# manoskary/analysisgnn

Hardware: AMD Instinct MI355X
Metric: subgraph-nodes/sec fwd+bwd, HybridGNN L=3 H=256 (higher is better)
Workload: dtype f32; 1 GPU; C2 (sampled, the batch a training step sees): HybridGNN L=3 H=256 out=128, 21 task heads, 32 neighbour-sampled subgraphs x (500 target notes + [5,5] hops) per GPU, per-hop counts passed (every layer trimmed); 16335 notes, 104099 edges per GPU; train step = fwd + objective (wloss) + bwd + allreduce + clip + AdamW, CSR rebuilt every step; hipGraph replay; workload_id=c2s, per_gpu_subgraphs=32, objective=wloss, parallelism=dp1, allreduce=none (one rank)

## Files before the change

analysisgnn_amd/_lib.py:

```python
from __future__ import annotations

import ctypes as C
import os
from typing import Optional, Sequence

import torch

from . import resident

_HERE = os.path.dirname(os.path.abspath(__file__))
LIB_PATH = os.path.join(_HERE, "libagnn_hip.so")
MAX_SEG = 32

SPMM_MEAN, SPMM_SKIP_SELF, SPMM_ACCUM = 1, 2, 4
INT32_MAX = 2 ** 31 - 1


class AgnnError(RuntimeError):
    pass


class CooSeg(C.Structure):
    _fields_ = [("row", C.c_void_p), ("col", C.c_void_p), ("etype", C.c_void_p),
                ("etype_code", C.c_int64), ("n_edges", C.c_int64), ("n_rows", C.c_int64)]
# ... 163 lines not shown
    "agnn_sample_members": (C.c_int, [C.c_void_p, C.c_int64, C.c_void_p, C.c_void_p, C.c_void_p, C.c_int32, C.c_int32, C.c_int32,
                                      C.POINTER(C.c_int32), C.c_int32, C.c_void_p, C.c_void_p, C.c_void_p, C.c_void_p]),
    "agnn_sample_compact_nodes": (C.c_int64, [C.POINTER(Sampler), C.POINTER(C.c_int32)]),
    "agnn_sample_compact": (C.c_int, [C.POINTER(Sampler), C.POINTER(C.c_int32), C.c_void_p, C.c_void_p, C.c_void_p]),
    "agnn_gather_rows_f32": (C.c_int, [C.c_void_p, C.c_int64, C.c_void_p, C.c_int64, C.c_int32, C.c_void_p, C.c_int64, C.c_void_p]),
    "agnn_gather_i64": (C.c_int, [C.c_void_p, C.c_int64, C.c_void_p, C.c_int64, C.c_int32, C.c_int64, C.c_void_p, C.c_int64, C.c_void_p]),
    "agnn_relt_fwd_f32": (C.c_int, [C.c_int, C.POINTER(ReltItem), C.c_int32, C.c_int32, C.c_int32, C.c_int64, C.c_void_p]),
    "agnn_relt_bwd_f32": (C.c_int, [C.c_int, C.POINTER(ReltItem), C.c_int32, C.c_int32, C.c_int32, C.c_int64, C.c_void_p]),
    "agnn_relt_dw_workspace_bytes": (C.c_size_t, [C.c_int, C.c_int32, C.c_int32, C.c_int32, C.c_int64]),
    "agnn_relt_dw_f32": (C.c_int, [C.c_int, C.POINTER(ReltItem), C.c_int32, C.c_int32, C.c_int32, C.c_int64, C.c_void_p, C.c_size_t,
                                  C.c_void_p]),
    "agnn_wgrad_batch_workspace_bytes": (C.c_size_t, [C.c_int32, C.POINTER(WgradItem)]),
    "agnn_wgrad_batch_f32": (C.c_int, [C.c_int32, C.POINTER(WgradItem), C.c_void_p, C.c_size_t, C.c_void_p]),
    "agnn_grad_epilogue_workspace_bytes": (C.c_size_t, [C.c_int32, C.POINTER(GradItem)]),
    "agnn_grad_epilogue_f32": (C.c_int, [C.c_int32, C.POINTER(GradItem), C.c_int32, C.POINTER(ColsumItem), C.c_void_p, C.c_size_t, C.c_void_p]),
    "agnn_gemm_nt_f32": (C.c_int, [C.c_void_p, C.c_int64, C.c_void_p, C.c_int64, C.c_void_p, C.c_int64, C.c_int32, C.c_int32, C.c_void_p,
                                   C.c_int64, C.c_void_p]),
    "agnn_gemm_nn_f32": (C.c_int, [C.c_void_p, C.c_int64, C.c_void_p, C.c_int64, C.c_void_p, C.c_int64, C.c_int32, C.c_int32, C.c_void_p,
                                   C.c_int64, C.c_void_p]),
    "agnn_gemm_nt2_f32": (C.c_int, [C.c_void_p, C.c_int64, C.c_int32, C.c_void_p, C.c_int64, C.c_int32, C.c_void_p, C.c_int64, C.c_void_p,
                                    C.c_int64, C.c_int32, C.c_void_p, C.c_int64, C.c_void_p]),
    "agnn_pool_cat_norm_f32": (C.c_int, [C.POINTER(Rel), C.c_void_p, C.c_int64, C.c_int64, C.c_int64, C.c_int32, C.c_int32, C.c_void_p,
                                         C.c_void_p, C.c_float, C.c_void_p, C.c_int64, C.c_void_p, C.c_int64, C.c_void_p, C.c_void_p,
                                         C.c_void_p, C.c_void_p]),
    "agnn_pool_cat_bwd_f32": (C.c_int, [C.POINTER(Rel), C.c_void_p, C.c_int64, C.c_void_p, C.c_int64, C.c_int64, C.c_int32, C.c_void_p,
                                        C.c_int64, C.c_void_p]),
    "agnn_absdiff_fwd_f32": (C.c_int, [C.c_void_p, C.c_void_p, C.c_void_p, C.c_int64, C.c_int64, C.c_int32, C.c_void_p, C.c_void_p, C.c_int64,
                                       C.c_void_p]),
    "agnn_absdiff_bwd_f32": (C.c_int, [C.c_void_p, C.c_void_p, C.c_void_p, C.c_int64, C.c_int64, C.c_int32, C.c_void_p, C.c_void_p, C.c_int64,
                                       C.c_int32, C.c_int32, C.c_void_p, C.c_int64, C.c_void_p]),
# ... 199 lines not shown
```

analysisgnn_amd/csrc/wgrad.hip:

```cpp
#include "agnn_common.h"

namespace {

typedef float f32x16 __attribute__((ext_vector_type(16)));

struct WgArgs {
  const float* dy;
  const float* x;
  int64_t ld_dy, ld_x;
  int32_t n, out_f, in_f;
  int32_t rows_per_slice;
  int32_t tiles_in;
  float* slab;
  float* slab_b;
  int32_t out_pad, in_pad;
};

__device__ __forceinline__ void wgrad_tile(const WgArgs& a, const int tile, const int slice) {
  const int lane = threadIdx.x & 63;
  const int wave = threadIdx.x >> 6;
  const int wm = wave >> 1, wn = wave & 1;
  const int to = tile / a.tiles_in, ti = tile - to * a.tiles_in;
  const int kk = lane >> 5, c32 = lane & 31;
  const int ocol = to * 128 + wm * 64 + 2 * c32;
// ... 480 lines not shown
  int32_t item, c0, c1;
};

bool spans_overlap(const EpiSpan& a, const EpiSpan& b) {
  const float* a_end = a.p + static_cast<int64_t>(a.rows - 1) * a.ld + a.cols;
  const float* b_end = b.p + static_cast<int64_t>(b.rows - 1) * b.ld + b.cols;
  if (a_end <= b.p || b_end <= a.p) return false;
  if (a.rows > 1 && b.rows > 1 && a.ld == b.ld) {
    int64_t r = (b.p - a.p) % a.ld;
    if (r < 0) r += a.ld;
    if (r >= a.cols && r + b.cols <= a.ld) return false;
  }
  return true;
}

}

static void epi_as_wgrad(int32_t n_items, const agnn_grad_item_t* items, agnn_wgrad_item_t* out) {
  for (int i = 0; i < n_items; ++i) {
    const agnn_grad_item_t& g = items[i];
    out[i] = agnn_wgrad_item_t{g.dy, g.x, nullptr, nullptr, g.ld_dy, g.ld_x, g.in_f, g.n, g.out_f, g.in_f};
  }
}

extern "C" size_t agnn_grad_epilogue_workspace_bytes(int32_t n_items, const agnn_grad_item_t* items) {
  if (n_items <= 0 || n_items > kWgBatchMax || !items) return 0;
  agnn_wgrad_item_t w[kWgBatchMax];
  epi_as_wgrad(n_items, items, w);
  return agnn_wgrad_batch_workspace_bytes(n_items, w);
}
// ... 5 lines not shown
  if (n_sums < 0 || n_sums > kEpiSumMax || (n_sums > 0 && !sums)) return fail(AGNN_EINVAL, "grad_epilogue: %d column sums (0 .. %d)", n_sums, kEpiSumMax);
  if (n_items == 0 && n_sums == 0) return AGNN_OK;
  BatchPlan bp;
  bp.n = 0;
  bp.total_floats = 0;
  float* ws = nullptr;
  if (n_items > 0) {
    agnn_wgrad_item_t w[kWgBatchMax];
    epi_as_wgrad(n_items, items, w);
    if (int rc = batch_plan(n_items, w, bp)) return rc;
    if (!workspace || workspace_bytes < bp.total_floats * sizeof(float) + 256) return fail(AGNN_ENOMEM, "grad_epilogue: workspace too small");
    ws = reinterpret_cast<float*>((reinterpret_cast<uintptr_t>(workspace) + 255) & ~uintptr_t{255});
  }
  static thread_local EpiSpan spans[kWgBatchMax * 2 * AGNN_PACK_MAX_SRC + 2 * kEpiSumMax];
  int n_spans = 0;
  for (int i = 0; i < n_items; ++i) {
    const agnn_grad_item_t& it = items[i];
    if ((it.out_f & 1) || (it.in_f & 1) || (it.ld_dy & 1) || (it.ld_x & 1)) return fail(AGNN_EALIGN, "grad_epilogue: item %d: widths and leading dimensions must be even", i);
    if (!it.dy || !it.x) return fail(AGNN_EINVAL, "grad_epilogue: item %d: null argument", i);
    if ((reinterpret_cast<uintptr_t>(it.dy) | reinterpret_cast<uintptr_t>(it.x)) & 7u) return fail(AGNN_EALIGN, "grad_epilogue: item %d: pointers must be 8-byte aligned", i);
    if (it.ld_dy < it.out_f || it.ld_x < it.in_f) return fail(AGNN_EINVAL, "grad_epilogue: item %d: leading dimension smaller than the width", i);
    if ((static_cast<int64_t>(bp.rps[i]) + 128) * (it.ld_dy > it.ld_x ? it.ld_dy : it.ld_x) * 4 >= (int64_t{1} << 32))
      return fail(AGNN_EINVAL, "grad_epilogue: item %d: a row slice (%d rows x ld) exceeds the kernel's 32-bit byte offsets", i, bp.rps[i]);
    if (it.n_dw < 0 || it.n_dw > AGNN_PACK_MAX_SRC || it.n_db < 0 || it.n_db > AGNN_PACK_MAX_SRC || it.n_dw + it.n_db == 0)
      return fail(AGNN_EINVAL, "grad_epilogue: item %d: %d weight and %d bias destinations (0 .. %d each, one at least)", i, it.n_dw, it.n_db, AGNN_PACK_MAX_SRC);
    for (int k = 0; k < it.n_dw; ++k) {
      const agnn_grad_dst_t& d = it.dw[k];
      const int cols = d.c1 - d.c0;
      if (!d.p || d.c0 < 0 || cols <= 0 || d.c1 > it.in_f || d.ld < cols || d.ld >= (int64_t{1} << 31))
        return fail(AGNN_EINVAL, "grad_epilogue: item %d: destination %d: columns [%d, %d) of %d, ld %lld", i, k, d.c0, d.c1, it.in_f, (long long)d.ld);
      if (reinterpret_cast<uintptr_t>(d.p) & 3u) return fail(AGNN_EALIGN, "grad_epilogue: item %d: destination %d is not a float pointer", i, k);
      if (!(cols & 1) && ((d.c0 & 1) || (d.ld & 1) || (reinterpret_cast<uintptr_t>(d.p) & 7u)))
        return fail(AGNN_EALIGN, "grad_epilogue: item %d: destination %d: an even column block needs an even c0, an even ld and an 8-byte aligned pointer", i, k);
      spans[n_spans++] = EpiSpan{d.p, d.ld, it.out_f, cols, i, d.c0, d.c1};
    }
    for (int k = 0; k < it.n_db; ++k) {
      if (!it.db[k]) return fail(AGNN_EINVAL, "grad_epilogue: item %d: null bias destination %d", i, k);
      if (reinterpret_cast<uintptr_t>(it.db[k]) & 3u) return fail(AGNN_EALIGN, "grad_epilogue: item %d: bias destination %d is not a float pointer", i, k);
      spans[n_spans++] = EpiSpan{it.db[k], it.out_f, 1, it.out_f, -1, 0, 0};
    }
  }
  for (int i = 0; i < n_sums; ++i) {
    const agnn_colsum_item_t& it = sums[i];
    if (it.n <= 0 || it.H <= 0 || (it.H & 3) || it.H > 2048 || !it.workspace || !it.dgamma || !it.dbeta)
      return fail(AGNN_EINVAL, "grad_epilogue: column sum %d: bad sizes or null argument", i);
    if (it.workspace_bytes < static_cast<size_t>(kEpiPartRows) * 2 * it.H * sizeof(float)) return fail(AGNN_ENOMEM, "grad_epilogue: column sum %d: workspace too small", i);
    if ((reinterpret_cast<uintptr_t>(it.dgamma) | reinterpret_cast<uintptr_t>(it.dbeta) | reinterpret_cast<uintptr_t>(it.workspace)) & 3u)
      return fail(AGNN_EALIGN, "grad_epilogue: column sum %d: misaligned", i);
    spans[n_spans++] = EpiSpan{it.dgamma, it.H, 1, it.H, -1, 0, 0};
    spans[n_spans++] = EpiSpan{it.dbeta, it.H, 1, it.H, -1, 0, 0};
  }
  for (int a = 0; a < n_spans; ++a)
    for (int c = a + 1; c < n_spans; ++c) {
      const EpiSpan &sa = spans[a], &sc = spans[c];
      if (sa.item >= 0 && sa.item == sc.item && sa.c0 == sc.c0 && sa.c1 == sc.c1 && sa.p == sc.p && sa.ld == sc.ld) continue;
      if (spans_overlap(sa, sc)) return fail(AGNN_EINVAL, "grad_epilogue: destinations %d and %d of the call overlap", a, c);
    }
  hipStream_t s = static_cast<hipStream_t>(stream_);
  if (n_items > 0) {
    WgBatch wb{};
    wb.n = n_items;
    int wg = 0;
    for (int i = 0; i < n_items; ++i) {
      const agnn_grad_item_t& it = items[i];
      const int out_pad = bp.tiles_out[i] * 128, in_pad = bp.tiles_in[i] * 128;
      wb.it[i] = WgArgs{it.dy, it.x, it.ld_dy, it.ld_x, static_cast<int32_t>(it.n), it.out_f, it.in_f, bp.rps[i], bp.tiles_in[i], ws + bp.slab_off[i],
                        it.n_db > 0 ? ws + bp.slabb_off[i] : nullptr, out_pad, in_pad};
      wb.tiles[i] = bp.tiles_out[i] * bp.tiles_in[i];
      wb.first[i] = wg;
      wg += wb.tiles[i] * bp.S[i];
    }
    wb.first[n_items] = wg;
// ... 2 lines not shown
  }
  int at = 0;
  do {
    EpiBatch eb{};
    int n = 0, n_rec = 0, n_db = 0, blocks = 0;
    while (at < n_items && n_rec + items[at].n_dw <= kEpiRecMax && n_db + items[at].n_db <= kEpiDbMax) {
      const agnn_grad_item_t& it = items[at];
      EpiItem& e = eb.it[n];
      e.slab = ws + bp.slab_off[at];
      e.slab_b = it.n_db > 0 ? ws + bp.slabb_off[at] : nullptr;
      e.S = bp.S[at];
      e.out_f = it.out_f;
      e.in_f = it.in_f;
      e.out_pad = bp.tiles_out[at] * 128;
      e.in_pad = bp.tiles_in[at] * 128;
      e.rec0 = static_cast<int16_t>(n_rec);
      for (int k = 0; k < it.n_dw; ++k) {
        const agnn_grad_dst_t& d = it.dw[k];
        eb.rec[n_rec++] = EpiRec{d.p, static_cast<int32_t>(d.ld), d.c0, d.c1, (d.c1 - d.c0) & 1};
      }
      e.rec1 = static_cast<int16_t>(n_rec);
      e.db0 = static_cast<int16_t>(n_db);
      for (int k = 0; k < it.n_db; ++k) eb.db[n_db++] = it.db[k];
      e.db1 = static_cast<int16_t>(n_db);
      eb.first[n] = blocks;
      int64_t rb = (static_cast<int64_t>(it.out_f) * (it.in_f >> 1) + 31) / 32;
      if (rb > 1024) rb = 1024;
      blocks += static_cast<int>(rb);
      ++n;
      ++at;
    }
    eb.n_items = n;
    if (at == n_items)
      for (int i = 0; i < n_sums; ++i) {
        const agnn_colsum_item_t& it = sums[i];
        int nb = static_cast<int>((it.n + 3) / 4);
        if (nb > kEpiPartRows) nb = kEpiPartRows;
        eb.sum[i] = EpiSum{static_cast<const float*>(it.workspace), it.dgamma, it.dbeta, nb, it.H};
        eb.first[n++] = blocks;
// ... 12 lines not shown
```

analysisgnn_amd/heads.py:

```python
from __future__ import annotations

from typing import Dict, List, Optional, Sequence, Tuple

import torch
import torch.nn as nn
import torch.nn.functional as F

from . import _lib, resident
from .fused import grouped_norm_act
from .linear import all_steal, defer, deferring, grad_slot_groups, leaf_refs, linear, mark_wgrad_async, slot_group, wgrad_stream
from .params import cat_rows, stack_rows


def fused_head_logits(clf_dict: nn.ModuleDict, x: torch.Tensor, tasks: Sequence[str]) -> Tuple[torch.Tensor, List[int]]:
    mods = [clf_dict[t] for t in tasks]
    T = len(mods)
    h2 = mods[0][0].out_features
    W1 = _cat_params([m[0].weight for m in mods])
    b1 = _cat_params([m[0].bias for m in mods])
    gamma = _cat_params([m[2].weight for m in mods], stack=True)
    beta = _cat_params([m[2].bias for m in mods], stack=True)
    offs = [0]
    for m in mods:
        offs.append(offs[-1] + m[3].out_features)
    b2 = _cat_params([m[3].bias for m in mods])
# ... 278 lines not shown
def multitask_cross_entropy(logits: torch.Tensor, offs: Sequence[int], labels: torch.Tensor, label_smoothing: float = 0.1,
                            ignore_index: int = -1) -> torch.Tensor:
    full = len(offs) > 1 and offs[0] == 0 and offs[-1] == logits.shape[1] and all(offs[i] < offs[i + 1] for i in range(len(offs) - 1))
    return _MultiTaskCE.apply(logits, labels, _offs_tensor(offs, logits.device), label_smoothing, ignore_index, full)


def _check_labels(labels: torch.Tensor, T: int, N: int) -> torch.Tensor:
    if labels.dtype != torch.int64:
        raise _lib.AgnnError(f"labels must be int64 (torch.long), got {labels.dtype}")
    if tuple(labels.shape) != (T, N):
        raise _lib.AgnnError(f"labels must have shape [T={T}, N={N}] (one row per task), got {tuple(labels.shape)}")
    return labels.contiguous()


FINAL_GRADIENTS = True


def unit_gradient(device) -> torch.Tensor:
    return resident.value(device, ("unit gradient",), lambda: torch.ones((), dtype=torch.float32, device=device))


class _TrainLoss(torch.autograd.Function):

    @staticmethod
    def forward(ctx, logits, labels, offs_t, feat, task_param, eps: float, ignore_index: int, lam: float, ce_scale: float):
        dev = _lib.require_gpu(logits, labels, offs_t, feat)
        if logits.dtype != torch.float32 or logits.stride(1) != 1:
            logits = logits.float().contiguous()
        if feat.dtype != torch.float32 or feat.stride(1) != 1:
            feat = feat.float().contiguous()
        N = logits.shape[0]
        T = offs_t.numel() - 1
        labels = _check_labels(labels, T, N)
        tp = None
        if task_param is not None:
            tp = task_param.detach().to(torch.float32).contiguous()
            if tp.numel() != T:
                raise _lib.AgnnError(f"task_param must have {T} entries, got {tp.numel()}")
        lib = _lib.load()
        ws = resident.scratch(dev, "train_loss", int(lib.agnn_train_loss_workspace_bytes()), zeroed=True)
        row_loss = torch.empty((T, N), dtype=torch.float32, device=dev)
        out = torch.empty((4 * T + 1,), dtype=torch.float32, device=dev)
        dlogits = torch.empty_like(logits)
        ctx.final = FINAL_GRADIENTS
        dfeat = None
        if ctx.final:
            dfeat = torch.empty_like(feat) if ctx.needs_input_grad[3] else None
            _lib.check(lib.agnn_train_loss_final_f32(logits.data_ptr(), logits.stride(0), offs_t.data_ptr(), T, labels.data_ptr(), N, float(eps),
                                                     int(ignore_index), feat.data_ptr(), feat.stride(0), feat.shape[1], float(lam),
                                                     _lib.ptr(tp), float(ce_scale), row_loss.data_ptr(), dlogits.data_ptr(), out.data_ptr(),
                                                     out[T:].data_ptr(), out[2 * T:].data_ptr(), out[2 * T + 1:].data_ptr(),
                                                     out[3 * T + 1:].data_ptr(), _lib.ptr(dfeat), dfeat.stride(0) if dfeat is not None else 0,
                                                     ws.data_ptr(), int(lib.agnn_train_loss_workspace_bytes()), _lib.stream_ptr(dev)),
                       "agnn_train_loss_final_f32")
        else:
            _lib.check(lib.agnn_train_loss_f32(logits.data_ptr(), logits.stride(0), offs_t.data_ptr(), T, labels.data_ptr(), N, float(eps),
                                               int(ignore_index), feat.data_ptr(), feat.stride(0), feat.shape[1], float(lam),
                                               _lib.ptr(tp), float(ce_scale), row_loss.data_ptr(), dlogits.data_ptr(), out.data_ptr(),
                                               out[T:].data_ptr(), out[2 * T:].data_ptr(), out[2 * T + 1:].data_ptr(),
                                               out[3 * T + 1:].data_ptr(), ws.data_ptr(), int(lib.agnn_train_loss_workspace_bytes()),
                                               _lib.stream_ptr(dev)), "agnn_train_loss_f32")
        ctx.save_for_backward(dlogits, offs_t, out, feat, *([dfeat] if dfeat is not None else []))
        ctx.lam = float(lam)
        ctx.T = T
        ctx.has_param = task_param is not None
        ctx.mark_non_differentiable(out)
        ctx.set_materialize_grads(False)
        return out[2 * T], out

    @staticmethod
    def backward(ctx, g, _g_parts):
        dlogits, offs_t, out, feat, *rest = ctx.saved_tensors
        dev = dlogits.device
        T = ctx.T
        want_param = ctx.has_param and ctx.needs_input_grad[4]
        if ctx.final:
            dfeat = rest[0] if rest else None
            if dfeat is None and ctx.needs_input_grad[3]:
                dfeat = (2.0 * ctx.lam / feat.numel()) * feat
            dparam = out[3 * T + 1:4 * T + 1] if want_param else None
            if g.data_ptr() == unit_gradient(dev).data_ptr():
                return dlogits, None, None, dfeat, dparam, None, None, None, None
            g = g.to(torch.float32)
            return (dlogits * g, None, None, dfeat * g if dfeat is not None else None, dparam * g if dparam is not None else None,
                    None, None, None, None)
        g = g.to(torch.float32).contiguous()
        dl = torch.empty_like(dlogits)
        dfeat = torch.empty_like(feat) if ctx.needs_input_grad[3] else None
        lib = _lib.load()
        _lib.check(lib.agnn_train_loss_bwd_f32(dlogits.data_ptr(), dlogits.stride(0), offs_t.data_ptr(), T, dlogits.shape[0],
                                               dlogits.shape[1], out[2 * T + 1:].data_ptr(), g.data_ptr(), dl.data_ptr(), dl.stride(0),
                                               feat.data_ptr(), feat.stride(0), feat.shape[1], ctx.lam, _lib.ptr(dfeat),
                                               dfeat.stride(0) if dfeat is not None else 0, _lib.stream_ptr(dev)),
                   "agnn_train_loss_bwd_f32")
        dparam = out[3 * T + 1:4 * T + 1] * g if want_param else None
# ... 52 lines not shown
```

analysisgnn_amd/linear.py:

```python
from __future__ import annotations

from typing import Optional

import torch
import torch.nn as nn
import torch.nn.functional as F

from . import _lib, resident

MIN_ROWS = 2048
MAX_OUT_IN = 512 * 1024
ENABLED = True


_WG = {"enabled": False, "scope": "all", "dirty": set()}


def enable_wgrad_overlap(flag: bool = True, scope="all") -> None:
    _WG["enabled"] = bool(flag)
    _WG["scope"] = scope if scope == "all" else frozenset([scope] if isinstance(scope, str) else scope)


def wgrad_overlap_enabled() -> bool:
    return _WG["enabled"]
# ... 363 lines not shown

    def tensors(self):
        if self.dsts is not None:
            return (self.dy, self.x, *[d for _, _, d in self.dsts], *self.db_dsts)
        return (self.dy, self.x, self.dw_out, self.db_out)

    def destinations(self):
        if self.dsts is not None:
            return self.dsts, self.db_dsts
        return [(0, self.x.shape[1], self.dw_out)], ((self.db_out,) if self.want_bias else ())

    def __call__(self):
        if self.dsts is None:
            weight_grad(self.dy, self.x, self.want_bias, dw_out=self.dw_out, db_out=self.db_out)
            return
        from .params import pack
        dw, db = weight_grad(self.dy, self.x, self.want_bias)
        items = [(d, [dw[:, c0:c1]]) for c0, c1, d in self.dsts] + [(d.view(1, -1), [db.view(1, -1)]) for d in self.db_dsts]
        pack(items, self.dy.device)


class ColsumItem:
    __slots__ = ("ws", "n", "H", "dgamma", "dbeta", "event")

    def __init__(self, ws, n, H, dgamma, dbeta):
        self.ws, self.n, self.H, self.dgamma, self.dbeta, self.event = ws, int(n), int(H), dgamma, dbeta, None

    def tensors(self):
        return (self.ws, self.dgamma, self.dbeta)

# ... 58 lines not shown
            group.append(it)
            products += 0 if joins else 1
        else:
            it()
    if group:
        run(group)


def _dst_ok(d: torch.Tensor, out_f: int, c0: int, c1: int) -> bool:
    cols = c1 - c0
    if d.dtype != torch.float32 or d.dim() != 2 or tuple(d.shape) != (out_f, cols) or d.stride(1) != 1 or d.stride(0) < cols:
        return False
    return d.data_ptr() % 4 == 0 if cols & 1 else (c0 % 2 == 0 and d.stride(0) % 2 == 0 and d.data_ptr() % 8 == 0)


def grad_epilogue(items, sums) -> None:
    lib = _lib.load()

    def fits(it):
        n, out_f = it.dy.shape
        in_f = it.x.shape[1]
        dsts, dbs = it.destinations()
        return (ENABLED and it.dy.is_cuda and it.dy.dim() == 2 and it.x.dim() == 2 and n >= MIN_ROWS and out_f * in_f <= MAX_OUT_IN and in_f % 2 == 0
                and _ok(it.dy) and _ok(it.x) and 0 < len(dsts) <= _lib.PACK_MAX_SRC and len(dbs) <= _lib.PACK_MAX_SRC
                and all(d is not None and _dst_ok(d, out_f, c0, c1) for c0, c1, d in dsts) and bool(dbs) == it.want_bias
                and all(d is not None and d.is_contiguous() and tuple(d.shape) == (out_f,) for d in dbs)
                and (it.dsts is not None or all(d.data_ptr() % 8 == 0 for d in dbs)))

    groups, group, products = [], [], 0
    for it in items:
        if fits(it):
            joins = it.follows and group and group[-1].dy is it.dy
            if group and ((products == _lib.WGRAD_BATCH_MAX and not joins) or len(group) == _lib.WGRAD_BATCH_MAX_ITEMS):
                groups.append(group)
                group, products, joins = [], 0, False
            group.append(it)
            products += 0 if joins else 1
        else:
            it()
    if group:
        groups.append(group)
    sums = list(sums)
    batched = [g for g in groups if len(g) > 1]
    for g in groups:
        if len(g) == 1:
            g[0]()
            continue
        take, sums = (sums[:_lib.GRAD_MAX_SUMS], sums[_lib.GRAD_MAX_SUMS:]) if g is batched[-1] else ([], sums)
        _epilogue_call(lib, g, take)
    while sums:
        _epilogue_call(lib, [], sums[:_lib.GRAD_MAX_SUMS])
        sums = sums[_lib.GRAD_MAX_SUMS:]


def _epilogue_call(lib, group, sums) -> None:
    dev = (group[0].dy if group else sums[0].ws).device
    arr = (_lib.GradItem * max(len(group), 1))()
    for a, it in zip(arr, group):
        dsts, dbs = it.destinations()
        a.dy, a.x = it.dy.data_ptr(), it.x.data_ptr()
        a.ld_dy, a.ld_x, a.n = it.dy.stride(0), it.x.stride(0), it.dy.shape[0]
        a.out_f, a.in_f = it.dy.shape[1], it.x.shape[1]
        a.n_dw, a.n_db = len(dsts), len(dbs)
        for k, (c0, c1, d) in enumerate(dsts):
            a.dw[k].p, a.dw[k].ld, a.dw[k].c0, a.dw[k].c1 = d.data_ptr(), (d.stride(0) if d.shape[0] > 1 else max(d.shape[1], d.stride(0))), c0, c1
        for k, d in enumerate(dbs):
            a.db[k] = d.data_ptr()
    sarr = (_lib.ColsumItem * max(len(sums), 1))()
    for a, it in zip(sarr, sums):
        a.workspace, a.workspace_bytes, a.n, a.H = it.ws.data_ptr(), it.ws.numel(), it.n, it.H
        a.dgamma, a.dbeta = it.dgamma.data_ptr(), it.dbeta.data_ptr()
    nws = int(lib.agnn_grad_epilogue_workspace_bytes(len(group), arr)) if group else 0
    ws = torch.empty(nws, dtype=torch.uint8, device=dev) if group else None
    _lib.check(lib.agnn_grad_epilogue_f32(len(group), arr, len(sums), sarr, _lib.ptr(ws), nws, _lib.stream_ptr(dev)), "agnn_grad_epilogue_f32")


def _leaf_slots(groups, out_f: int, in_f: int, odd_ok: bool = False):
    if groups is None or not groups[0]:
        return None

    def ok(v):
        dw, db = v
# ... 218 lines not shown
```

analysisgnn_amd/params.py:

```python
from __future__ import annotations

from typing import List, Sequence, Tuple

import torch

from . import _lib
from .linear import all_steal, defer, deferring, mark_wgrad_async, wgrad_stream


def pack(items: Sequence[Tuple[torch.Tensor, Sequence[torch.Tensor]]], device) -> None:
    arr = (_lib.PackItem * len(items))()
    for i, (dst, srcs) in enumerate(items):
        if len(srcs) > _lib.PACK_MAX_SRC:
            raise _lib.AgnnError(f"pack: {len(srcs)} sources (max {_lib.PACK_MAX_SRC})")
        rows, cols = dst.shape
        ld_src = (srcs[0].stride(0) if rows > 1 else max(cols, 1)) if srcs else max(cols, 1)
        for t in (dst, *srcs):
            if t.dtype != torch.float32 or t.dim() != 2 or (cols > 1 and t.stride(1) != 1) or tuple(t.shape) != (rows, cols):
                raise _lib.AgnnError("pack: fp32 2-D pieces of one shape with unit inner stride expected")
        for k, t in enumerate(srcs):
            if rows > 1 and t.stride(0) != ld_src:
                raise _lib.AgnnError("pack: the sources of an item must share their row stride")
            arr[i].src[k] = t.data_ptr()
        arr[i].dst = dst.data_ptr()
# ... 55 lines not shown
                for r in range(R):
                    items.append((G_r[r], [dW_r_]))
            pack(items, dev)
        off_chain = ctx.leaves and all_steal(ctx.param_refs)
        if off_chain and deferring(dW_l):
            defer(fan_out, dev)
        else:
            with wgrad_stream(dev, dW_l, db, dW_r, active=off_chain):
                fan_out()
        g_lb = (*G_l.unbind(0), *G_b.unbind(0)) if sl_l is None else tuple(sl_l)
        g_r = G_r.unbind(0) if sl_r is None else tuple(sl_r)
        del sl_l, sl_r
        return (None, None, *g_lb, *g_r)


class _SageOperandsCat(torch.autograd.Function):

    @staticmethod
    def forward(ctx, R: int, with_l: bool, box, *params):
        w_l, b_l, w_r = params[:R], params[R:2 * R], params[2 * R:]
        dev = _lib.require_gpu(*params)
        ctx.box = box
        out_f, in_f = w_r[0].shape
        nl = R if with_l else 0
        W = torch.empty((out_f, (nl + 1) * in_f), dtype=torch.float32, device=dev)
        b = torch.empty((out_f,), dtype=torch.float32, device=dev)
        items = [(W[:, r * in_f:(r + 1) * in_f], [w_l[r].detach()]) for r in range(nl)]
        items.append((b.view(1, -1), [t.detach().view(1, -1) for t in b_l]))
        items.append((W[:, nl * in_f:], [t.detach() for t in w_r]))
        pack(items, dev)
        ctx.R, ctx.nl = R, nl
        ctx.shape = (out_f, in_f)
        ctx.leaves = all(t.is_leaf for t in params)
        ctx.param_refs = tuple(params)
        return W, b

    @staticmethod
    def backward(ctx, dW, db):
        R, nl = ctx.R, ctx.nl
        out_f, in_f = ctx.shape
        dev = dW.device
        slots = ctx.box.pop("slots", None) if ctx.box is not None else None
        if slots is not None:
            by = {id(p): v for p, v in zip(ctx.box["leaves"], slots)}
            w_l, b_l, w_r = ctx.param_refs[:R], ctx.param_refs[R:2 * R], ctx.param_refs[2 * R:]
            g_l = [by[id(p)] for p in w_l] if nl else list(torch.zeros((R, out_f, in_f), dtype=torch.float32, device=dev).unbind(0))
            out = (None, None, None, *g_l, *[by[id(p)] for p in b_l], *[by[id(p)] for p in w_r])
            del slots, by, g_l
            return out
        G_l = torch.empty((nl, out_f, in_f), dtype=torch.float32, device=dev)
        G_b = torch.empty((R, out_f), dtype=torch.float32, device=dev)
        G_r = torch.empty((R, out_f, in_f), dtype=torch.float32, device=dev)
        if not nl:
            G_l = torch.zeros((R, out_f, in_f), dtype=torch.float32, device=dev)

        def fan_out():
            dW_, db_ = _lib.f32c(dW), db.contiguous()
            items = []
            for r in range(R):
                if r < nl:
                    items.append((G_l[r], [dW_[:, r * in_f:(r + 1) * in_f]]))
                items.append((G_b[r].view(1, -1), [db_.view(1, -1)]))
                items.append((G_r[r], [dW_[:, nl * in_f:]]))
            pack(items, dev)
        off_chain = ctx.leaves and all_steal(ctx.param_refs)
        if off_chain and deferring(dW):
            defer(fan_out, dev)
        else:
            with wgrad_stream(dev, dW, db, active=off_chain):
                fan_out()
        return (None, None, None, *G_l.unbind(0), *G_b.unbind(0), *G_r.unbind(0))


def sage_operands_cat(w_l: List[torch.Tensor], b_l: List[torch.Tensor], w_r: List[torch.Tensor], with_l: bool = True):
    R = len(w_l)
    ok = (w_l[0].is_cuda and R <= _lib.PACK_MAX_SRC and all(t is not None for t in b_l)
          and all(t.shape == w_l[0].shape and t.is_contiguous() for t in (*w_l, *w_r)))
    if not ok:
        return None
    leaves_ok = all(t.is_leaf for t in (*w_l, *b_l, *w_r))
    box = None
    if leaves_ok:
        in_f = w_r[0].shape[1]
        nl = R if with_l else 0
        box = {"uses": 0, "leaves": (*(w_l if with_l else ()), *b_l, *w_r), "b": tuple(b_l),
               "w": tuple([(r * in_f, (r + 1) * in_f, w_l[r]) for r in range(nl)] + [(nl * in_f, (nl + 1) * in_f, t) for t in w_r])}
# ... 75 lines not shown
```

include/agnn.h:

```cpp
#ifndef AGNN_H_
#define AGNN_H_

#include <stddef.h>
#include <stdint.h>

#ifdef __cplusplus
extern "C" {
#endif

typedef void* agnn_stream_t;

#define AGNN_OK        0
#define AGNN_EINVAL  (-22)
#define AGNN_EALIGN  (-14)
#define AGNN_ENOMEM  (-12)
#define AGNN_ERUNTIME (-5)

#define AGNN_MAX_SEG 32

const char* agnn_last_error(void);
int agnn_version(void);

typedef struct {
  const int64_t* row;
// ... 220 lines not shown
  int64_t ld;
  int32_t c0, c1;
} agnn_grad_dst_t;
typedef struct {
  const float* dy;
  const float* x;
  int64_t ld_dy, ld_x, n;
  int32_t out_f, in_f;
  int32_t n_dw, n_db;
  agnn_grad_dst_t dw[AGNN_PACK_MAX_SRC];
  float* db[AGNN_PACK_MAX_SRC];
} agnn_grad_item_t;
size_t agnn_grad_epilogue_workspace_bytes(int32_t n_items, const agnn_grad_item_t* items );
int agnn_grad_epilogue_f32(int32_t n_items, const agnn_grad_item_t* items , int32_t n_sums,
                           const agnn_colsum_item_t* sums , void* workspace, size_t workspace_bytes, agnn_stream_t stream);

#define AGNN_GATHER_MAX_ITEMS 128
typedef struct {
  float* dst;
  const float* src;
  int64_t n;
} agnn_gather_item_t;
int agnn_gather_f32(int32_t n_items, const agnn_gather_item_t* items , agnn_stream_t stream);

int agnn_debug_stamp(uint64_t* slot , agnn_stream_t stream);

#define AGNN_EMBED_MAX_TABLES 4
int agnn_embed_cat_fwd_f32(const float* x, int64_t ld_x, int32_t in_x, int64_t n_rows, int32_t n_tab,
                           const int64_t* const* idx, const float* const* tables, const int32_t* vocab, int32_t dim,
                           float* out, int64_t ld_out, agnn_stream_t stream);
// ... 226 lines not shown
```

Before: 5.769 million subgraph-nodes/s.

## Write lone weight gradients, task-param grads and zero grads directly into grad slots

Adds a single-item wgrad entry point that computes the weight gradient and reduces slices straight into the destination columns and bias, instead of producing dW/db and then packing them. Task-parameter gradients from the final loss kernel are written into the stolen grad slot. Zero gradients for unused SAGE weights are written in place with a gather/zero kernel rather than allocating fresh zero tensors. This removes intermediate buffers and copy kernels in backward, at the cost of more aliasing logic around grad slots, with a clone fallback when a grad already exists.

```diff
diff --git a/analysisgnn_amd/_lib.py b/analysisgnn_amd/_lib.py
--- a/analysisgnn_amd/_lib.py
+++ b/analysisgnn_amd/_lib.py
@@ -201,6 +201,7 @@
     "agnn_wgrad_batch_f32": (C.c_int, [C.c_int32, C.POINTER(WgradItem), C.c_void_p, C.c_size_t, C.c_void_p]),
     "agnn_grad_epilogue_workspace_bytes": (C.c_size_t, [C.c_int32, C.POINTER(GradItem)]),
     "agnn_grad_epilogue_f32": (C.c_int, [C.c_int32, C.POINTER(GradItem), C.c_int32, C.POINTER(ColsumItem), C.c_void_p, C.c_size_t, C.c_void_p]),
+    "agnn_wgrad_dst_f32": (C.c_int, [C.POINTER(GradItem), C.c_void_p, C.c_size_t, C.c_void_p]),
     "agnn_gemm_nt_f32": (C.c_int, [C.c_void_p, C.c_int64, C.c_void_p, C.c_int64, C.c_void_p, C.c_int64, C.c_int32, C.c_int32, C.c_void_p,
                                    C.c_int64, C.c_void_p]),
     "agnn_gemm_nn_f32": (C.c_int, [C.c_void_p, C.c_int64, C.c_void_p, C.c_int64, C.c_void_p, C.c_int64, C.c_int32, C.c_int32, C.c_void_p,
diff --git a/analysisgnn_amd/csrc/wgrad.hip b/analysisgnn_amd/csrc/wgrad.hip
--- a/analysisgnn_amd/csrc/wgrad.hip
+++ b/analysisgnn_amd/csrc/wgrad.hip
@@ -518,6 +518,95 @@
   return true;
 }
 
+int epi_check_item(const char* who, int i, const agnn_grad_item_t& it, int rps, EpiSpan* spans, int& n_spans) {
+  using namespace agnn;
+  if ((it.out_f & 1) || (it.in_f & 1) || (it.ld_dy & 1) || (it.ld_x & 1)) return fail(AGNN_EALIGN, "%s: item %d: widths and leading dimensions must be even", who, i);
+  if (!it.dy || !it.x) return fail(AGNN_EINVAL, "%s: item %d: null argument", who, i);
+  if ((reinterpret_cast<uintptr_t>(it.dy) | reinterpret_cast<uintptr_t>(it.x)) & 7u) return fail(AGNN_EALIGN, "%s: item %d: pointers must be 8-byte aligned", who, i);
+  if (it.ld_dy < it.out_f || it.ld_x < it.in_f) return fail(AGNN_EINVAL, "%s: item %d: leading dimension smaller than the width", who, i);
+  if ((static_cast<int64_t>(rps) + 128) * (it.ld_dy > it.ld_x ? it.ld_dy : it.ld_x) * 4 >= (int64_t{1} << 32))
+    return fail(AGNN_EINVAL, "%s: item %d: a row slice (%d rows x ld) exceeds the kernel's 32-bit byte offsets", who, i, rps);
+  if (it.n_dw < 0 || it.n_dw > AGNN_PACK_MAX_SRC || it.n_db < 0 || it.n_db > AGNN_PACK_MAX_SRC || it.n_dw + it.n_db == 0)
+    return fail(AGNN_EINVAL, "%s: item %d: %d weight and %d bias destinations (0 .. %d each, one at least)", who, i, it.n_dw, it.n_db, AGNN_PACK_MAX_SRC);
+  for (int k = 0; k < it.n_dw; ++k) {
+    const agnn_grad_dst_t& d = it.dw[k];
+    const int cols = d.c1 - d.c0;
+    if (!d.p || d.c0 < 0 || cols <= 0 || d.c1 > it.in_f || d.ld < cols || d.ld >= (int64_t{1} << 31))
+      return fail(AGNN_EINVAL, "%s: item %d: destination %d: columns [%d, %d) of %d, ld %lld", who, i, k, d.c0, d.c1, it.in_f, (long long)d.ld);
+    if (reinterpret_cast<uintptr_t>(d.p) & 3u) return fail(AGNN_EALIGN, "%s: item %d: destination %d is not a float pointer", who, i, k);
+    if (!(cols & 1) && ((d.c0 & 1) || (d.ld & 1) || (reinterpret_cast<uintptr_t>(d.p) & 7u)))
+      return fail(AGNN_EALIGN, "%s: item %d: destination %d: an even column block needs an even c0, an even ld and an 8-byte aligned pointer", who, i, k);
+    spans[n_spans++] = EpiSpan{d.p, d.ld, it.out_f, cols, i, d.c0, d.c1};
+  }
+  for (int k = 0; k < it.n_db; ++k) {
+    if (!it.db[k]) return fail(AGNN_EINVAL, "%s: item %d: null bias destination %d", who, i, k);
+    if (reinterpret_cast<uintptr_t>(it.db[k]) & 3u) return fail(AGNN_EALIGN, "%s: item %d: bias destination %d is not a float pointer", who, i, k);
+    spans[n_spans++] = EpiSpan{it.db[k], it.out_f, 1, it.out_f, -1, 0, 0};
+  }
+  return AGNN_OK;
+}
+
+int epi_check_overlaps(const char* who, const EpiSpan* spans, int n_spans) {
+  for (int a = 0; a < n_spans; ++a)
+    for (int c = a + 1; c < n_spans; ++c) {
+      const EpiSpan &sa = spans[a], &sc = spans[c];
+      if (sa.item >= 0 && sa.item == sc.item && sa.c0 == sc.c0 && sa.c1 == sc.c1 && sa.p == sc.p && sa.ld == sc.ld) continue;
+      if (spans_overlap(sa, sc)) return agnn::fail(AGNN_EINVAL, "%s: destinations %d and %d of the call overlap", who, a, c);
+    }
+  return AGNN_OK;
+}
+
+void epi_fill_item(EpiBatch& eb, EpiItem& e, const agnn_grad_item_t& it, int& n_rec, int& n_db) {
+  e.rec0 = static_cast<int16_t>(n_rec);
+  for (int k = 0; k < it.n_dw; ++k) {
+    const agnn_grad_dst_t& d = it.dw[k];
+    eb.rec[n_rec++] = EpiRec{d.p, static_cast<int32_t>(d.ld), d.c0, d.c1, (d.c1 - d.c0) & 1};
+  }
+  e.rec1 = static_cast<int16_t>(n_rec);
+  e.db0 = static_cast<int16_t>(n_db);
+  for (int k = 0; k < it.n_db; ++k) eb.db[n_db++] = it.db[k];
+  e.db1 = static_cast<int16_t>(n_db);
+}
+
+}
+
+extern "C" int agnn_wgrad_dst_f32(const agnn_grad_item_t* item, void* workspace, size_t workspace_bytes, agnn_stream_t stream_) {
+  using namespace agnn;
+  if (!item) return fail(AGNN_EINVAL, "wgrad_dst: null item");
+  const agnn_grad_item_t& it = *item;
+  if (it.n <= 0 || it.n >= (int64_t{1} << 31) || it.out_f <= 0 || it.in_f <= 0) return fail(AGNN_EINVAL, "wgrad_dst: bad sizes n=%lld out=%d in=%d", (long long)it.n, it.out_f, it.in_f);
+  const Plan p = make_plan(it.n, it.out_f, it.in_f);
+  EpiSpan spans[2 * AGNN_PACK_MAX_SRC];
+  int n_spans = 0;
+  if (int rc = epi_check_item("wgrad_dst", 0, it, p.rows_per_slice, spans, n_spans)) return rc;
+  if (int rc = epi_check_overlaps("wgrad_dst", spans, n_spans)) return rc;
+  const size_t need = agnn_wgrad_workspace_bytes(it.n, it.out_f, it.in_f);
+  if (!workspace || workspace_bytes < need) return fail(AGNN_ENOMEM, "wgrad_dst: workspace %zu < %zu bytes", workspace_bytes, need);
+  float* slab = reinterpret_cast<float*>((reinterpret_cast<uintptr_t>(workspace) + 255) & ~uintptr_t{255});
+  float* slab_b = slab + static_cast<size_t>(p.S) * p.out_pad * p.in_pad;
+  WgArgs a{it.dy, it.x, it.ld_dy, it.ld_x, static_cast<int32_t>(it.n), it.out_f, it.in_f, p.rows_per_slice, p.tiles_in, slab,
+           it.n_db > 0 ? slab_b : nullptr, p.out_pad, p.in_pad};
+  hipStream_t s = static_cast<hipStream_t>(stream_);
+  hipLaunchKernelGGL(k_wgrad, dim3(p.tiles_out * p.tiles_in, p.S), dim3(256), 0, s, a);
+  if (int rc = check_launch("wgrad_dst")) return rc;
+  EpiBatch eb{};
+  EpiItem& e = eb.it[0];
+  e.slab = slab;
+  e.slab_b = it.n_db > 0 ? slab_b : nullptr;
+  e.S = p.S;
+  e.out_f = it.out_f;
+  e.in_f = it.in_f;
+  e.out_pad = p.out_pad;
+  e.in_pad = p.in_pad;
+  int n_rec = 0, n_db = 0;
+  epi_fill_item(eb, e, it, n_rec, n_db);
+  int64_t blocks = (static_cast<int64_t>(it.out_f) * (it.in_f >> 1) + 31) / 32;
+  if (blocks > 4096) blocks = 4096;
+  eb.first[0] = 0;
+  eb.first[1] = static_cast<int32_t>(blocks);
+  eb.n_items = eb.n_all = 1;
+  hipLaunchKernelGGL(k_grad_epilogue, dim3(static_cast<unsigned>(blocks)), dim3(256), 0, s, eb);
+  return check_launch("wgrad_dst(reduce)");
 }
 
 static void epi_as_wgrad(int32_t n_items, const agnn_grad_item_t* items, agnn_wgrad_item_t* out) {
@@ -553,32 +642,8 @@
   }
   static thread_local EpiSpan spans[kWgBatchMax * 2 * AGNN_PACK_MAX_SRC + 2 * kEpiSumMax];
   int n_spans = 0;
-  for (int i = 0; i < n_items; ++i) {
-    const agnn_grad_item_t& it = items[i];
-    if ((it.out_f & 1) || (it.in_f & 1) || (it.ld_dy & 1) || (it.ld_x & 1)) return fail(AGNN_EALIGN, "grad_epilogue: item %d: widths and leading dimensions must be even", i);
-    if (!it.dy || !it.x) return fail(AGNN_EINVAL, "grad_epilogue: item %d: null argument", i);
-    if ((reinterpret_cast<uintptr_t>(it.dy) | reinterpret_cast<uintptr_t>(it.x)) & 7u) return fail(AGNN_EALIGN, "grad_epilogue: item %d: pointers must be 8-byte aligned", i);
-    if (it.ld_dy < it.out_f || it.ld_x < it.in_f) return fail(AGNN_EINVAL, "grad_epilogue: item %d: leading dimension smaller than the width", i);
-    if ((static_cast<int64_t>(bp.rps[i]) + 128) * (it.ld_dy > it.ld_x ? it.ld_dy : it.ld_x) * 4 >= (int64_t{1} << 32))
-      return fail(AGNN_EINVAL, "grad_epilogue: item %d: a row slice (%d rows x ld) exceeds the kernel's 32-bit byte offsets", i, bp.rps[i]);
-    if (it.n_dw < 0 || it.n_dw > AGNN_PACK_MAX_SRC || it.n_db < 0 || it.n_db > AGNN_PACK_MAX_SRC || it.n_dw + it.n_db == 0)
-      return fail(AGNN_EINVAL, "grad_epilogue: item %d: %d weight and %d bias destinations (0 .. %d each, one at least)", i, it.n_dw, it.n_db, AGNN_PACK_MAX_SRC);
-    for (int k = 0; k < it.n_dw; ++k) {
-      const agnn_grad_dst_t& d = it.dw[k];
-      const int cols = d.c1 - d.c0;
-      if (!d.p || d.c0 < 0 || cols <= 0 || d.c1 > it.in_f || d.ld < cols || d.ld >= (int64_t{1} << 31))
-        return fail(AGNN_EINVAL, "grad_epilogue: item %d: destination %d: columns [%d, %d) of %d, ld %lld", i, k, d.c0, d.c1, it.in_f, (long long)d.ld);
-      if (reinterpret_cast<uintptr_t>(d.p) & 3u) return fail(AGNN_EALIGN, "grad_epilogue: item %d: destination %d is not a float pointer", i, k);
-      if (!(cols & 1) && ((d.c0 & 1) || (d.ld & 1) || (reinterpret_cast<uintptr_t>(d.p) & 7u)))
-        return fail(AGNN_EALIGN, "grad_epilogue: item %d: destination %d: an even column block needs an even c0, an even ld and an 8-byte aligned pointer", i, k);
-      spans[n_spans++] = EpiSpan{d.p, d.ld, it.out_f, cols, i, d.c0, d.c1};
-    }
-    for (int k = 0; k < it.n_db; ++k) {
-      if (!it.db[k]) return fail(AGNN_EINVAL, "grad_epilogue: item %d: null bias destination %d", i, k);
-      if (reinterpret_cast<uintptr_t>(it.db[k]) & 3u) return fail(AGNN_EALIGN, "grad_epilogue: item %d: bias destination %d is not a float pointer", i, k);
-      spans[n_spans++] = EpiSpan{it.db[k], it.out_f, 1, it.out_f, -1, 0, 0};
-    }
-  }
+  for (int i = 0; i < n_items; ++i)
+    if (int rc = epi_check_item("grad_epilogue", i, items[i], bp.rps[i], spans, n_spans)) return rc;
   for (int i = 0; i < n_sums; ++i) {
     const agnn_colsum_item_t& it = sums[i];
     if (it.n <= 0 || it.H <= 0 || (it.H & 3) || it.H > 2048 || !it.workspace || !it.dgamma || !it.dbeta)
@@ -589,12 +654,7 @@
     spans[n_spans++] = EpiSpan{it.dgamma, it.H, 1, it.H, -1, 0, 0};
     spans[n_spans++] = EpiSpan{it.dbeta, it.H, 1, it.H, -1, 0, 0};
   }
-  for (int a = 0; a < n_spans; ++a)
-    for (int c = a + 1; c < n_spans; ++c) {
-      const EpiSpan &sa = spans[a], &sc = spans[c];
-      if (sa.item >= 0 && sa.item == sc.item && sa.c0 == sc.c0 && sa.c1 == sc.c1 && sa.p == sc.p && sa.ld == sc.ld) continue;
-      if (spans_overlap(sa, sc)) return fail(AGNN_EINVAL, "grad_epilogue: destinations %d and %d of the call overlap", a, c);
-    }
+  if (int rc = epi_check_overlaps("grad_epilogue", spans, n_spans)) return rc;
   hipStream_t s = static_cast<hipStream_t>(stream_);
   if (n_items > 0) {
     WgBatch wb{};
@@ -627,15 +687,7 @@
       e.in_f = it.in_f;
       e.out_pad = bp.tiles_out[at] * 128;
       e.in_pad = bp.tiles_in[at] * 128;
-      e.rec0 = static_cast<int16_t>(n_rec);
-      for (int k = 0; k < it.n_dw; ++k) {
-        const agnn_grad_dst_t& d = it.dw[k];
-        eb.rec[n_rec++] = EpiRec{d.p, static_cast<int32_t>(d.ld), d.c0, d.c1, (d.c1 - d.c0) & 1};
-      }
-      e.rec1 = static_cast<int16_t>(n_rec);
-      e.db0 = static_cast<int16_t>(n_db);
-      for (int k = 0; k < it.n_db; ++k) eb.db[n_db++] = it.db[k];
-      e.db1 = static_cast<int16_t>(n_db);
+      epi_fill_item(eb, e, it, n_rec, n_db);
       eb.first[n] = blocks;
       int64_t rb = (static_cast<int64_t>(it.out_f) * (it.in_f >> 1) + 31) / 32;
       if (rb > 1024) rb = 1024;
diff --git a/analysisgnn_amd/heads.py b/analysisgnn_amd/heads.py
--- a/analysisgnn_amd/heads.py
+++ b/analysisgnn_amd/heads.py
@@ -8,7 +8,8 @@
 
 from . import _lib, resident
 from .fused import grouped_norm_act
-from .linear import all_steal, defer, deferring, grad_slot_groups, leaf_refs, linear, mark_wgrad_async, slot_group, wgrad_stream
+from .linear import (_steals, all_steal, defer, deferring, grad_slot_groups, grad_slot_of, grad_slots, leaf_refs, linear, mark_wgrad_async,
+                     slot_group, wgrad_stream)
 from .params import cat_rows, stack_rows
 
 
@@ -317,6 +318,7 @@
 
 
 FINAL_GRADIENTS = True
+TASK_GRAD_IN_PLACE = True
 
 
 def unit_gradient(device) -> torch.Tensor:
@@ -347,13 +349,20 @@
         dlogits = torch.empty_like(logits)
         ctx.final = FINAL_GRADIENTS
         dfeat = None
+        slot = None
+        if (TASK_GRAD_IN_PLACE and ctx.final and task_param is not None and ctx.needs_input_grad[4] and task_param.is_leaf
+                and task_param.dtype == torch.float32 and _steals(task_param)):
+            slot = grad_slots([task_param])
+        ctx.param_ref = task_param if slot is not None else None
+        dparam_ptr = slot[0].data_ptr() if slot is not None else out[3 * T + 1:].data_ptr()
+        del slot
         if ctx.final:
             dfeat = torch.empty_like(feat) if ctx.needs_input_grad[3] else None
             _lib.check(lib.agnn_train_loss_final_f32(logits.data_ptr(), logits.stride(0), offs_t.data_ptr(), T, labels.data_ptr(), N, float(eps),
                                                      int(ignore_index), feat.data_ptr(), feat.stride(0), feat.shape[1], float(lam),
                                                      _lib.ptr(tp), float(ce_scale), row_loss.data_ptr(), dlogits.data_ptr(), out.data_ptr(),
                                                      out[T:].data_ptr(), out[2 * T:].data_ptr(), out[2 * T + 1:].data_ptr(),
-                                                     out[3 * T + 1:].data_ptr(), _lib.ptr(dfeat), dfeat.stride(0) if dfeat is not None else 0,
+                                                     dparam_ptr, _lib.ptr(dfeat), dfeat.stride(0) if dfeat is not None else 0,
                                                      ws.data_ptr(), int(lib.agnn_train_loss_workspace_bytes()), _lib.stream_ptr(dev)),
                        "agnn_train_loss_final_f32")
         else:
@@ -382,6 +391,10 @@
             if dfeat is None and ctx.needs_input_grad[3]:
                 dfeat = (2.0 * ctx.lam / feat.numel()) * feat
             dparam = out[3 * T + 1:4 * T + 1] if want_param else None
+            if want_param and ctx.param_ref is not None:
+                dparam = grad_slot_of(ctx.param_ref)
+                if ctx.param_ref.grad is not None:
+                    dparam = dparam.clone()
             if g.data_ptr() == unit_gradient(dev).data_ptr():
                 return dlogits, None, None, dfeat, dparam, None, None, None, None
             g = g.to(torch.float32)
diff --git a/analysisgnn_amd/linear.py b/analysisgnn_amd/linear.py
--- a/analysisgnn_amd/linear.py
+++ b/analysisgnn_amd/linear.py
@@ -401,6 +401,15 @@
         if self.dsts is None:
             weight_grad(self.dy, self.x, self.want_bias, dw_out=self.dw_out, db_out=self.db_out)
             return
+        if LONE_IN_PLACE and _epilogue_fits(self):
+            lib = _lib.load()
+            arr = (_lib.GradItem * 1)()
+            _fill_grad_item(arr[0], self)
+            n, out_f = self.dy.shape
+            nws = int(lib.agnn_wgrad_workspace_bytes(n, out_f, self.x.shape[1]))
+            ws = torch.empty(nws, dtype=torch.uint8, device=self.dy.device)
+            _lib.check(lib.agnn_wgrad_dst_f32(arr, ws.data_ptr(), nws, _lib.stream_ptr(self.dy.device)), "agnn_wgrad_dst_f32")
+            return
         from .params import pack
         dw, db = weight_grad(self.dy, self.x, self.want_bias)
         items = [(d, [dw[:, c0:c1]]) for c0, c1, d in self.dsts] + [(d.view(1, -1), [db.view(1, -1)]) for d in self.db_dsts]
@@ -489,19 +498,35 @@
     return d.data_ptr() % 4 == 0 if cols & 1 else (c0 % 2 == 0 and d.stride(0) % 2 == 0 and d.data_ptr() % 8 == 0)
 
 
+LONE_IN_PLACE = True
+
+
+def _epilogue_fits(it) -> bool:
+    n, out_f = it.dy.shape
+    in_f = it.x.shape[1]
+    dsts, dbs = it.destinations()
+    return (ENABLED and it.dy.is_cuda and it.dy.dim() == 2 and it.x.dim() == 2 and n >= MIN_ROWS and out_f * in_f <= MAX_OUT_IN and in_f % 2 == 0
+            and _ok(it.dy) and _ok(it.x) and 0 < len(dsts) <= _lib.PACK_MAX_SRC and len(dbs) <= _lib.PACK_MAX_SRC
+            and all(d is not None and _dst_ok(d, out_f, c0, c1) for c0, c1, d in dsts) and bool(dbs) == it.want_bias
+            and all(d is not None and d.is_contiguous() and tuple(d.shape) == (out_f,) for d in dbs)
+            and (it.dsts is not None or all(d.data_ptr() % 8 == 0 for d in dbs)))
+
+
+def _fill_grad_item(a, it) -> None:
+    dsts, dbs = it.destinations()
+    a.dy, a.x = it.dy.data_ptr(), it.x.data_ptr()
+    a.ld_dy, a.ld_x, a.n = it.dy.stride(0), it.x.stride(0), it.dy.shape[0]
+    a.out_f, a.in_f = it.dy.shape[1], it.x.shape[1]
+    a.n_dw, a.n_db = len(dsts), len(dbs)
+    for k, (c0, c1, d) in enumerate(dsts):
+        a.dw[k].p, a.dw[k].ld, a.dw[k].c0, a.dw[k].c1 = d.data_ptr(), (d.stride(0) if d.shape[0] > 1 else max(d.shape[1], d.stride(0))), c0, c1
+    for k, d in enumerate(dbs):
+        a.db[k] = d.data_ptr()
+
+
 def grad_epilogue(items, sums) -> None:
     lib = _lib.load()
-
-    def fits(it):
-        n, out_f = it.dy.shape
-        in_f = it.x.shape[1]
-        dsts, dbs = it.destinations()
-        return (ENABLED and it.dy.is_cuda and it.dy.dim() == 2 and it.x.dim() == 2 and n >= MIN_ROWS and out_f * in_f <= MAX_OUT_IN and in_f % 2 == 0
-                and _ok(it.dy) and _ok(it.x) and 0 < len(dsts) <= _lib.PACK_MAX_SRC and len(dbs) <= _lib.PACK_MAX_SRC
-                and all(d is not None and _dst_ok(d, out_f, c0, c1) for c0, c1, d in dsts) and bool(dbs) == it.want_bias
-                and all(d is not None and d.is_contiguous() and tuple(d.shape) == (out_f,) for d in dbs)
-                and (it.dsts is not None or all(d.data_ptr() % 8 == 0 for d in dbs)))
-
+    fits = _epilogue_fits
     groups, group, products = [], [], 0
     for it in items:
         if fits(it):
@@ -532,15 +557,7 @@
     dev = (group[0].dy if group else sums[0].ws).device
     arr = (_lib.GradItem * max(len(group), 1))()
     for a, it in zip(arr, group):
-        dsts, dbs = it.destinations()
-        a.dy, a.x = it.dy.data_ptr(), it.x.data_ptr()
-        a.ld_dy, a.ld_x, a.n = it.dy.stride(0), it.x.stride(0), it.dy.shape[0]
-        a.out_f, a.in_f = it.dy.shape[1], it.x.shape[1]
-        a.n_dw, a.n_db = len(dsts), len(dbs)
-        for k, (c0, c1, d) in enumerate(dsts):
-            a.dw[k].p, a.dw[k].ld, a.dw[k].c0, a.dw[k].c1 = d.data_ptr(), (d.stride(0) if d.shape[0] > 1 else max(d.shape[1], d.stride(0))), c0, c1
-        for k, d in enumerate(dbs):
-            a.db[k] = d.data_ptr()
+        _fill_grad_item(a, it)
     sarr = (_lib.ColsumItem * max(len(sums), 1))()
     for a, it in zip(sarr, sums):
         a.workspace, a.workspace_bytes, a.n, a.H = it.ws.data_ptr(), it.ws.numel(), it.n, it.H
diff --git a/analysisgnn_amd/params.py b/analysisgnn_amd/params.py
--- a/analysisgnn_amd/params.py
+++ b/analysisgnn_amd/params.py
@@ -5,7 +5,7 @@
 import torch
 
 from . import _lib
-from .linear import all_steal, defer, deferring, mark_wgrad_async, wgrad_stream
+from .linear import all_steal, defer, deferring, grad_slots, mark_wgrad_async, wgrad_stream
 
 
 def pack(items: Sequence[Tuple[torch.Tensor, Sequence[torch.Tensor]]], device) -> None:
@@ -93,6 +93,21 @@
         return (None, None, *g_lb, *g_r)
 
 
+ZERO_IN_PLACE = True
+
+
+def _zero_grads(ps, shape, dev) -> list:
+    ps = list(ps)
+    views = grad_slots(ps) if (ZERO_IN_PLACE and all(p.is_leaf for p in ps) and all_steal(ps)) else None
+    if views is None:
+        return list(torch.zeros(shape, dtype=torch.float32, device=dev).unbind(0))
+    arr = (_lib.GatherItem * len(views))()
+    for a, v in zip(arr, views):
+        a.dst, a.src, a.n = v.data_ptr(), None, v.numel()
+    _lib.check(_lib.load().agnn_gather_f32(len(views), arr, _lib.stream_ptr(dev)), "agnn_gather_f32")
+    return views
+
+
 class _SageOperandsCat(torch.autograd.Function):
 
     @staticmethod
@@ -123,15 +138,16 @@
         if slots is not None:
             by = {id(p): v for p, v in zip(ctx.box["leaves"], slots)}
             w_l, b_l, w_r = ctx.param_refs[:R], ctx.param_refs[R:2 * R], ctx.param_refs[2 * R:]
-            g_l = [by[id(p)] for p in w_l] if nl else list(torch.zeros((R, out_f, in_f), dtype=torch.float32, device=dev).unbind(0))
+            g_l = [by[id(p)] for p in w_l] if nl else _zero_grads(w_l, (R, out_f, in_f), dev)
             out = (None, None, None, *g_l, *[by[id(p)] for p in b_l], *[by[id(p)] for p in w_r])
             del slots, by, g_l
             return out
         G_l = torch.empty((nl, out_f, in_f), dtype=torch.float32, device=dev)
         G_b = torch.empty((R, out_f), dtype=torch.float32, device=dev)
         G_r = torch.empty((R, out_f, in_f), dtype=torch.float32, device=dev)
+        g_l = None
         if not nl:
-            G_l = torch.zeros((R, out_f, in_f), dtype=torch.float32, device=dev)
+            g_l = _zero_grads(ctx.param_refs[:R], (R, out_f, in_f), dev)
 
         def fan_out():
             dW_, db_ = _lib.f32c(dW), db.contiguous()
@@ -148,7 +164,7 @@
         else:
             with wgrad_stream(dev, dW, db, active=off_chain):
                 fan_out()
-        return (None, None, None, *G_l.unbind(0), *G_b.unbind(0), *G_r.unbind(0))
+        return (None, None, None, *(G_l.unbind(0) if g_l is None else g_l), *G_b.unbind(0), *G_r.unbind(0))
 
 
 def sage_operands_cat(w_l: List[torch.Tensor], b_l: List[torch.Tensor], w_r: List[torch.Tensor], with_l: bool = True):
diff --git a/include/agnn.h b/include/agnn.h
--- a/include/agnn.h
+++ b/include/agnn.h
@@ -258,6 +258,7 @@
 size_t agnn_grad_epilogue_workspace_bytes(int32_t n_items, const agnn_grad_item_t* items );
 int agnn_grad_epilogue_f32(int32_t n_items, const agnn_grad_item_t* items , int32_t n_sums,
                            const agnn_colsum_item_t* sums , void* workspace, size_t workspace_bytes, agnn_stream_t stream);
+int agnn_wgrad_dst_f32(const agnn_grad_item_t* item , void* workspace, size_t workspace_bytes, agnn_stream_t stream);
 
 #define AGNN_GATHER_MAX_ITEMS 128
 typedef struct {
```

New measurement: 5.782 million subgraph-nodes/s, median of 6. No clear change (+0.2%).
